# actionml/universal-recommender

Hardware: NVIDIA H100
Metric: CCO train events/sec to indicator model (higher is better)
Workload: dtype int32+f64

## Files before the change

### universal_recommender_b200/csrc/cco_api.cu

```cuda
#include <cuda_runtime.h>
#include <dlfcn.h>
#include <stdarg.h>
#include <stdio.h>
#include <stdlib.h>
#include <string.h>

#include <algorithm>
#include <charconv>
#include <cmath>
#include <functional>
#include <cub/cub.cuh>
#include <nvtx3/nvToolsExt.h>
#include <condition_variable>
#include <mutex>
#include <string>
#include <thread>
#include <unordered_map>
#include <vector>

#include "../../include/cco_b200.h"
#include "cco_kernels.cuh"
#include "cco_sampler.cuh"
#include "cco_format.cuh"
#include "cco_strings.cuh"
// ... 382 lines not shown
  c->launches++;
  ar.release(tmp);
  ar.release(kb.Alternate());
  ar.release(vb.Alternate());
  *k = kb.Current();
  *v = vb.Current();
  return CCO_OK;
}
static int bits_for(long long n) {
  int b = 1;
  while ((1LL << b) < n) ++b;
  return b;
}

static int keys_to_csr(cco_ctx *c, Arena &ar, unsigned long long *k0, unsigned long long *k1, long long n, int bits, long long n_valid,
                       long long n_rows, int32_t *col, long long *rp, long long *n_unique) {
  cudaStream_t s = c->stream;
  cub::DoubleBuffer<unsigned long long> db(k0, k1);
  size_t tb = 0;
  CK(cub::DeviceRadixSort::SortKeys(nullptr, tb, db, n, 0, bits, s));
  void *tmp;
  CKR(ar.alloc((char **)&tmp, tb));
  CK(cub::DeviceRadixSort::SortKeys(tmp, tb, db, n, 0, bits, s));
  ar.release(tmp);
  unsigned long long *sorted = db.Current(), *other = db.Alternate();
  uint32_t *flag, *pos;
  CKR(ar.alloc(&flag, n_valid + 1));
  CKR(ar.alloc(&pos, n_valid + 1));
  CK(cudaMemsetAsync(flag + n_valid, 0, 4, s));
  k_unique_flags<<<grid_for(n_valid, 256, c->sm_count), 256, 0, s>>>(n_valid, sorted, flag);
  CKR(exclusive_sum(c, ar, flag, pos, n_valid + 1));
  uint32_t nuq = 0;
  CKR(mail_fetch(c, &nuq, pos + n_valid, 4));
  k_unique_scatter<<<grid_for(n_valid, 256, c->sm_count), 256, 0, s>>>(n_valid, sorted, flag, pos, other, col);
  CKR(mail_wait(c));
  k_rowptr_from_keys<<<grid_for(n_rows + 1, 256, c->sm_count), 256, 0, s>>>(n_rows, nuq, other, rp);
  c->launches += 3;
  ar.release(flag);
  ar.release(pos);
  *n_unique = nuq;
  return CCO_OK;
}

static int canonicalize_device(cco_ctx *c, Arena &ar, DevRaw &m) {
  if (m.nnz == 0) return CCO_OK;
  unsigned long long *k0, *k1;
  CKR(ar.alloc(&k0, m.nnz));
  CKR(ar.alloc(&k1, m.nnz));
  k_expand_keys<<<grid_for(m.n_rows * kSG, 256, c->sm_count), 256, 0, c->stream>>>(m.n_rows, m.rp, m.col, k0);
  c->launches++;
  long long n_unique = 0;
  CKR(keys_to_csr(c, ar, k0, k1, m.nnz, 32 + bits_for(m.n_rows), m.nnz, m.n_rows, m.col + m.q_base, m.rp, &n_unique));
  m.col += m.q_base;
  m.q_base = 0;
  m.nnz = n_unique;
  CK(cudaGetLastError());
  ar.release(k0);
  ar.release(k1);
  return CCO_OK;
}

struct HeavyRows {
  int32_t *list = nullptr;
  int *n = nullptr;
};
static int list_heavy_rows(cco_ctx *c, Arena &ar, const DevRaw &raw, HeavyRows *h) {
  CKR(ar.alloc(&h->list, std::max<long long>(raw.n_rows, 1)));
  CKR(ar.alloc(&h->n, 1));
  CK(cudaMemsetAsync(h->n, 0, 4, c->stream));
  if (raw.n_rows > 0) {
    k_list_heavy_rows<<<grid_for(raw.n_rows, 256, c->sm_count), 256, 0, c->stream>>>(raw.n_rows, raw.rp, h->list, h->n);
    c->launches++;
  }
  return CCO_OK;
}
static void launch_check(cco_ctx *c, const DevRaw &raw, const HeavyRows &h, int *flags) {
  if (raw.n_rows <= 0) return;
  const long long q_lo = raw.q_base, q_hi = raw.q_base + raw.nnz;
  k_check_rows<kSG><<<grid_for(raw.n_rows * kSG, 256, c->sm_count), 256, 0, c->stream>>>(raw.n_rows, raw.n_cols, raw.rp, raw.col, q_lo, q_hi,
                                                                                       nullptr, nullptr, flags);
  k_check_rows<32><<<c->sm_count * 4, 256, 0, c->stream>>>(raw.n_rows, raw.n_cols, raw.rp, raw.col, q_lo, q_hi, h.list, h.n, flags);
  c->launches += 2;
}
struct SampleScratch {
  unsigned long long *col_thr = nullptr;
  uint8_t *keep = nullptr;
};
static int sample_scratch(cco_ctx *c, Arena &ar, const DevRaw &raw, const int32_t *raw_counts, int32_t m, SampleScratch *sc) {
  CKR(ar.alloc(&sc->col_thr, std::max<int32_t>(raw.n_cols, 1)));
  CKR(ar.alloc(&sc->keep, std::max<long long>(raw.nnz, 1)));
  if (raw.n_cols > 0) {
    k_col_thresholds<<<grid_for(raw.n_cols, 256, c->sm_count, 4), 256, 0, c->stream>>>(raw.n_cols, raw_counts, m, sc->col_thr);
    c->launches++;
  }
  return CCO_OK;
}
static void launch_count(cco_ctx *c, const DevRaw &raw, const SampleScratch &sc, int32_t m, int32_t seed, uint32_t flags, const int *bad,
                         uint32_t *kept, int32_t *new_counts) {
  if (raw.n_rows <= 0 || raw.nnz <= 0) return;
  const long long q_lo = raw.q_base, q_hi = raw.q_base + raw.nnz;
  const long long n_chunks = (raw.nnz + kSampleChunk - 1) / kSampleChunk;
  k_sample_count<<<grid_for(n_chunks * 32, 256, c->sm_count), 256, 0, c->stream>>>(raw.n_rows, raw.row_base, raw.rp, raw.col, raw.n_cols, q_lo, q_hi,
                                                                                  sc.col_thr, m, seed, flags, bad, kept, new_counts, sc.keep);
  c->launches++;
}
static int launch_write(cco_ctx *c, Arena &ar, const DevRaw &raw, const SampleScratch &sc, int32_t *dst) {
  if (raw.n_rows <= 0 || raw.nnz <= 0) return CCO_OK;
  long long *n_sel;
  CKR(ar.alloc(&n_sel, 1));
  size_t tb = 0;
  CK(cub::DeviceSelect::Flagged(nullptr, tb, raw.col + raw.q_base, sc.keep, dst, n_sel, (long long)raw.nnz, c->stream));
  void *tmp;
  CKR(ar.alloc((char **)&tmp, tb));
  CK(cub::DeviceSelect::Flagged(tmp, tb, raw.col + raw.q_base, sc.keep, dst, n_sel, (long long)raw.nnz, c->stream));
  ar.release(tmp);
  c->launches += 2;
  return CCO_OK;
}

constexpr int kHistCopies = 16;
static bool hist_fits_smem(const cco_ctx *c, int32_t n_cols) { return ((size_t)n_cols + 1) / 2 * 4 <= c->smem_optin; }
static int count_raw_columns(cco_ctx *c, Arena &ar, const std::vector<DevRaw> &raw, const std::vector<long long> &col_off, const cudaEvent_t *ready,
                             int *verdict, int32_t **counts_out) {
  cudaStream_t s = c->stream;
  const int n_mats = (int)raw.size();
  const long long total_cols = col_off[n_mats];
  const long long copy_stride = std::max<long long>(total_cols, 1);
  bool copies = false;
  for (int i = 0; i < n_mats; ++i) copies = copies || (raw[i].n_rows > 0 && !hist_fits_smem(c, raw[i].n_cols));
  const int n_copies = copies ? kHistCopies : 1;
  int32_t *counts;
  CKR(ar.alloc(&counts, (size_t)copy_stride * n_copies));
  CK(cudaMemsetAsync(counts, 0, sizeof(int32_t) * (size_t)copy_stride * n_copies, s));
  *counts_out = counts;
  std::vector<int> fit;
  for (int i = 0; i < n_mats; ++i)
    if (raw[i].n_rows > 0 && hist_fits_smem(c, raw[i].n_cols)) fit.push_back(i);
  for (size_t b0 = 0; b0 < fit.size(); b0 += kHistSegs) {
    const size_t b1 = std::min(fit.size(), b0 + kHistSegs);
    HistBatch hb{};
    long long nnz_sum = 0;
    int32_t max_cols = 0;
    for (size_t t = b0; t < b1; ++t) {
      nnz_sum += raw[fit[t]].nnz;
      max_cols = std::max(max_cols, raw[fit[t]].n_cols);
    }
    const size_t smem = ((size_t)max_cols + 1) / 2 * 4;
    const int per_sm = std::max(1, std::min<int>(2048 / kHistThreads, (int)(c->smem_optin / std::max<size_t>(smem + 1024, 1))));
    const long long target = (long long)c->sm_count * per_sm;
    for (size_t t = b0; t < b1; ++t) {
      const int i = fit[t];
      if (ready) CK(cudaStreamWaitEvent(s, ready[i], 0));
      const long long share = nnz_sum > 0 ? (target * raw[i].nnz + nnz_sum - 1) / nnz_sum : 1;
      const long long need = (raw[i].nnz + kHistMinEntries - 1) / kHistMinEntries;
      HistSeg &g = hb.seg[hb.n++];
      g.col = raw[i].col + raw[i].q_base;
      g.rp = raw[i].rp;
      g.nnz = raw[i].nnz;
      g.n_rows = raw[i].n_rows;
      g.q_lo = raw[i].q_base;
      g.q_hi = raw[i].q_base + raw[i].nnz;
      g.counts = counts + col_off[i];
      g.verdict = verdict ? verdict + 2 * i : nullptr;
      g.n_cols = raw[i].n_cols;
      g.cta0 = hb.cta_end;
      hb.cta_end += (int32_t)std::max(1LL, std::min(share, need));
    }
    CK(cudaFuncSetAttribute(k_col_counts_smem, cudaFuncAttributeMaxDynamicSharedMemorySize, (int)smem));
    k_col_counts_smem<<<hb.cta_end, kHistThreads, smem, s>>>(hb);
    c->launches++;
  }
  for (int i = 0; i < n_mats && copies; ++i) {
    if (raw[i].n_rows == 0 || hist_fits_smem(c, raw[i].n_cols)) continue;
    if (ready) CK(cudaStreamWaitEvent(s, ready[i], 0));
    int *v = verdict ? verdict + 2 * i : nullptr;
    if (v) {
      k_check_row_ptr<<<grid_for(raw[i].n_rows, 256, c->sm_count), 256, 0, s>>>(raw[i].n_rows, raw[i].rp, raw[i].q_base, raw[i].q_base + raw[i].nnz, v);
      c->launches++;
    }
    if (raw[i].nnz > 0) {
      k_col_histogram_flat<true><<<grid_for(raw[i].nnz, 256, c->sm_count), 256, 0, s>>>(raw[i].nnz, raw[i].col + raw[i].q_base, raw[i].n_cols,
                                                                                       counts + col_off[i], kHistCopies, copy_stride, v);
      c->launches++;
    }
  }
  if (copies) {
    k_sum_copies<<<grid_for(total_cols, 256, c->sm_count), 256, 0, s>>>(total_cols, kHistCopies, copy_stride, counts);
    c->launches++;
  }
  if (ready)
    for (int i = 0; i < n_mats; ++i) CK(cudaStreamWaitEvent(s, ready[i], 0));
  return CCO_OK;
}

static int nccl_check(int rc, const char *what) {
  if (rc != 0) return set_error(CCO_E_NCCL, "%s: %s", what, g_nccl.GetErrorString(rc));
  return CCO_OK;
}

static int downsample_all(cco_ctx *c, Arena &ar, const std::vector<DevRaw> &raw, const int *d_check , long long U,
                          const int32_t *raw_counts, int32_t *marg_all, const std::vector<long long> &col_off,
                          const cco_indicator_params_t *params, int32_t seed, uint32_t flags, std::vector<DevMat> &dm,
                          const cudaEvent_t *stage_ev ) {
  cudaStream_t s = c->stream;
  const int W = c->world, r = c->rank, n_mats = (int)raw.size();
  const long long S = (U + W - 1) / W;
  std::vector<uint32_t *> kept(n_mats, nullptr);
  std::vector<SampleScratch> sc(n_mats);
  for (int i = 0; i < n_mats; ++i) {
    DevMat *out = &dm[i];
    out->n_rows = U;
    out->n_cols = raw[i].n_cols;
    out->marg = marg_all + col_off[i];
    CKR(ar.alloc(&kept[i], (size_t)(W * S + 1)));
    CKR(ar.alloc(&out->rp, U + 1));
    CK(cudaMemsetAsync(kept[i], 0, sizeof(uint32_t) * (size_t)(W * S + 1), s));
    CKR(sample_scratch(c, ar, raw[i], raw_counts + col_off[i], params[i].max_interactions, &sc[i]));
    launch_count(c, raw[i], sc[i], params[i].max_interactions, seed, flags, d_check + 2 * i, kept[i], out->marg);
  }
  CK(cudaEventRecord(stage_ev[0], s));
  if (W > 1) {
    if (S > 0) {
      g_nccl.GroupStart();
      for (int i = 0; i < n_mats; ++i) {
        int rc = g_nccl.AllGather(kept[i] + (size_t)r * S, kept[i], (size_t)S, kNcclUint32, c->comm, s);
        if (rc != 0) { g_nccl.GroupEnd(); return nccl_check(rc, "ncclAllGather(kept counts)"); }
      }
      CKR(nccl_check(g_nccl.GroupEnd(), "ncclGroupEnd(kept counts)"));
    }
    if (col_off[n_mats] > 0)
      CKR(nccl_check(g_nccl.AllReduce(marg_all, marg_all, (size_t)col_off[n_mats], kNcclInt32, kNcclSum, c->comm, s), "ncclAllReduce(marginals)"));
  }
  std::vector<uint32_t> edge((size_t)n_mats * (W + 1), 0);
  for (int i = 0; i < n_mats; ++i) {
    CKR(exclusive_sum(c, ar, kept[i], dm[i].rp, U + 1));
    ar.release(kept[i]);
    if (W > 1)
      for (int q = 0; q <= W; ++q) CKR(mail_fetch(c, &edge[(size_t)i * (W + 1) + q], dm[i].rp + std::min<long long>((long long)q * S, U), 4));
  }
  CK(cudaEventRecord(stage_ev[1], s));
  if (W > 1) CKR(mail_wait(c));
  std::vector<long long> cap(n_mats, 0);
  std::vector<int32_t *> gathered(n_mats, nullptr);
  for (int i = 0; i < n_mats; ++i) {
    if (W == 1) {
      CKR(ar.alloc(&dm[i].col, std::max<long long>(raw[i].nnz, 1)));
      CKR(launch_write(c, ar, raw[i], sc[i], dm[i].col));
    } else {
      for (int q = 0; q < W; ++q) cap[i] = std::max<long long>(cap[i], (long long)edge[(size_t)i * (W + 1) + q + 1] - edge[(size_t)i * (W + 1) + q]);
      CKR(ar.alloc(&dm[i].col, std::max<long long>(edge[(size_t)i * (W + 1) + W], 1)));
      if (cap[i] > 0) {
        CKR(ar.alloc(&gathered[i], (size_t)(cap[i] * W)));
        CKR(launch_write(c, ar, raw[i], sc[i], gathered[i] + (size_t)r * cap[i]));
      }
    }
    ar.release(sc[i].col_thr);
    ar.release(sc[i].keep);
  }
  CK(cudaEventRecord(stage_ev[2], s));
  if (W > 1) {
    g_nccl.GroupStart();
    for (int i = 0; i < n_mats; ++i) {
      if (!gathered[i]) continue;
      int rc = g_nccl.AllGather(gathered[i] + (size_t)r * cap[i], gathered[i], (size_t)cap[i], kNcclInt32, c->comm, s);
      if (rc != 0) { g_nccl.GroupEnd(); return nccl_check(rc, "ncclAllGather(column blocks)"); }
    }
    CKR(nccl_check(g_nccl.GroupEnd(), "ncclGroupEnd(column blocks)"));
    for (int i = 0; i < n_mats; ++i) {
      if (!gathered[i]) continue;
      dim3 grid((unsigned)std::max(1, std::min(c->sm_count * 8 / W, 1024)), (unsigned)W);
      k_pack_blocks<<<grid, 256, 0, s>>>(W, S, U, cap[i], dm[i].rp, gathered[i], dm[i].col);
      c->launches++;
      ar.release(gathered[i]);
    }
  }
  CK(cudaEventRecord(stage_ev[3], s));
  CK(cudaGetLastError());
  return CCO_OK;
}


struct BinCfg {
  int group;
  int slots;
  int cap;
  int cbuf;
  int caux, keep_max, final_max;
  bool dense;
  bool bitmap;
  bool sorted;
  int bm_words;
  size_t region;
  size_t smem;
  int ctas_per_sm;
};

static int next_pow2(int x) {
  int p = 1;
  while (p < x) p <<= 1;
  return p;
}

template <int GROUP>
static int launch_rows_t(cco_ctx *c, const RowArgs &a, BinCfg &cfg, cudaStream_t st) {
  constexpr int CTA = GROUP == 32 ? 64 : GROUP;
  int occ = 1;
  void (*kern)(const RowArgs) = cfg.dense ? k_rows<GROUP, true> : k_rows<GROUP, false>;
  if constexpr (GROUP == 512 || GROUP == 256)
    if (cfg.bitmap) kern = k_rows<GROUP, false, true>;
  if constexpr (GROUP == 32)
    if (cfg.sorted) kern = k_rows<32, false, false, true>;
  CK(cudaFuncSetAttribute(kern, cudaFuncAttributeMaxDynamicSharedMemorySize, (int)cfg.smem));
  CK(cudaOccupancyMaxActiveBlocksPerMultiprocessor(&occ, kern, CTA, cfg.smem));
  kern<<<c->sm_count * std::max(occ, 1) * 4, CTA, cfg.smem, st>>>(a);
  cfg.ctas_per_sm = occ;
  c->launches++;
  CK(cudaGetLastError());
  return CCO_OK;
}
static int launch_rows(cco_ctx *c, const RowArgs &a, BinCfg &cfg, cudaStream_t st) {
  switch (cfg.group) {
    case 1024: return launch_rows_t<1024>(c, a, cfg, st);
    case 512: return launch_rows_t<512>(c, a, cfg, st);
    case 256: return launch_rows_t<256>(c, a, cfg, st);
    case 128: return launch_rows_t<128>(c, a, cfg, st);
    case 32: return launch_rows_t<32>(c, a, cfg, st);
  }
  return set_error(CCO_E_INVALID_ARG, "internal: bad bin config");
}

static BinCfg make_cfg(cco_ctx *c, int group, int want_slots, int top_k, int n_cols_b) {
  BinCfg f;
  const int groups = group == 32 ? 2 : 1;
  f.group = group;
  f.final_max = next_pow2(top_k);
  f.cbuf = next_pow2(top_k + std::max(group, 128) + (group == 32 ? 64 : 0));
  if (group == 32 && top_k + 32 <= 96) f.cbuf = 128;
  f.keep_max = std::max(f.final_max, (f.cbuf - group) / 2);
  f.caux = group == 32 ? 0 : f.keep_max;
  size_t fixed = (size_t)(f.cbuf + f.caux) * 16 + 2 * 256 + 512 + 1024 + (size_t)(group / 32) * 256;
  size_t avail = (c->smem_optin - 1024) / groups;
// ... 5101 lines not shown
    if (len[i] < 1 || len[i] > 32) return set_error(CCO_E_CUDA, "text %lld has length %d", (long long)i, len[i]);
    memcpy(bytes + offsets[i], slot.data() + 32 * (size_t)i, (size_t)len[i]);
    offsets[i + 1] = offsets[i] + len[i];
  }
  return CCO_OK;
}

int cco_debug_downsample(cco_ctx_t *c, const cco_csr_t *m, int32_t max_interactions, int32_t seed, uint32_t flags,
                         int64_t **row_ptr, int32_t **col_idx, int32_t *raw_col_counts, int32_t *new_col_counts) {
  if (!c || !m || !row_ptr || !col_idx) return set_error(CCO_E_INVALID_ARG, "null argument");
  if (c->world != 1 || !c->members.empty()) return set_error(CCO_E_UNSUPPORTED, "debug entries need a single-GPU context");
  cco_indicator_params_t prm = {max_interactions, 1, 0, 0.0};
  CKR(validate_host(1, m, &prm));
  CK(cudaSetDevice(c->device));
  mail_reset(c);
  c->ev_timing_used = c->ev_plain_used = 0;
  cco_dataset *ds = nullptr;
  CKR(dataset_upload(c, 1, m, flags, &ds));
  struct DG { cco_dataset *d; ~DG() { dataset_release(d); } } dg{ds};
  Arena ar(c->stream);
  Prepared p;
  CKR(prepare(c, ar, ds, &prm, seed, flags, &p));
  const DevMat &dm = p.dm[0];
  std::vector<uint32_t> rp32((size_t)m->n_rows + 1);
  CK(cudaMemcpyAsync(rp32.data(), dm.rp, sizeof(uint32_t) * rp32.size(), cudaMemcpyDeviceToHost, c->stream));
  if (raw_col_counts && m->n_cols > 0)
    CK(cudaMemcpyAsync(raw_col_counts, p.raw_counts, sizeof(int32_t) * (size_t)m->n_cols, cudaMemcpyDeviceToHost, c->stream));
  if (new_col_counts && m->n_cols > 0)
    CK(cudaMemcpyAsync(new_col_counts, dm.marg, sizeof(int32_t) * (size_t)m->n_cols, cudaMemcpyDeviceToHost, c->stream));
  CK(cudaStreamSynchronize(c->stream));
  CK(cudaGetLastError());
  size_t nnz = rp32[m->n_rows];
  int64_t *rp = (int64_t *)malloc(sizeof(int64_t) * rp32.size());
  int32_t *ci = (int32_t *)calloc(std::max<size_t>(nnz, 1), sizeof(int32_t));
  if (!rp || !ci) return set_error(CCO_E_OOM, "malloc failed");
  for (size_t i = 0; i < rp32.size(); ++i) rp[i] = rp32[i];
  const size_t n_copy = std::min<size_t>(nnz, (size_t)ds->nnz[0]);
  if (n_copy) CK(cudaMemcpy(ci, dm.col, sizeof(int32_t) * n_copy, cudaMemcpyDeviceToHost));
  *row_ptr = rp;
  *col_idx = ci;
  return CCO_OK;
}

int cco_debug_downsample_block(cco_ctx_t *c, const cco_csr_t *m, int64_t row_lo, int64_t row_hi, const int32_t *raw_col_counts,
                               int32_t max_interactions, int32_t seed, uint32_t flags, int64_t *kept_per_row, int32_t **col_idx,
                               int32_t *new_col_counts) {
  if (!c || !m || !col_idx || (m->n_rows > 0 && !kept_per_row) || (m->n_cols > 0 && (!raw_col_counts || !new_col_counts)))
    return set_error(CCO_E_INVALID_ARG, "null argument");
  if (c->world != 1 || !c->members.empty()) return set_error(CCO_E_UNSUPPORTED, "debug entries need a single-GPU context");
  cco_indicator_params_t prm = {max_interactions, 1, 0, 0.0};
  CKR(validate_host(1, m, &prm));
  if (row_lo < 0 || row_hi < row_lo || row_hi > m->n_rows)
    return set_error(CCO_E_INVALID_ARG, "rows [%lld, %lld) outside [0, %lld)", (long long)row_lo, (long long)row_hi, (long long)m->n_rows);
  CK(cudaSetDevice(c->device));
  mail_reset(c);
  cudaStream_t s = c->stream;
  cco_dataset *ds = nullptr;
  CKR(dataset_upload(c, 1, m, flags, &ds));
  struct DG { cco_dataset *d; ~DG() { dataset_release(d); } } dg{ds};
  Arena ar(s);
  const long long U = ds->n_users;
  const int32_t width = std::max<int32_t>(m->n_cols, 1);
  long long q[2] = {0, 0};
  CK(cudaMemcpyAsync(&q[0], ds->rp[0] + row_lo, sizeof(long long), cudaMemcpyDeviceToHost, s));
  CK(cudaMemcpyAsync(&q[1], ds->rp[0] + row_hi, sizeof(long long), cudaMemcpyDeviceToHost, s));
  CK(cudaStreamSynchronize(s));
  DevRaw blk;
  blk.n_rows = row_hi - row_lo;
  blk.row_base = row_lo;
  blk.n_cols = m->n_cols;
  blk.q_base = q[0];
  blk.nnz = q[1] - q[0];
  blk.rp = ds->rp[0] + row_lo;
  blk.col = ds->col[0];
  int32_t *counts, *marg, *dst;
  uint32_t *kept;
  CKR(ar.alloc(&counts, width));
  CKR(ar.alloc(&marg, width));
  CKR(ar.alloc(&kept, U + 1));
  CKR(ar.alloc(&dst, std::max<long long>(blk.nnz, 1)));
  if (m->n_cols > 0) CK(cudaMemcpyAsync(counts, raw_col_counts, sizeof(int32_t) * (size_t)m->n_cols, cudaMemcpyHostToDevice, s));
  CK(cudaMemsetAsync(marg, 0, sizeof(int32_t) * (size_t)width, s));
  CK(cudaMemsetAsync(kept, 0, sizeof(uint32_t) * ((size_t)U + 1), s));
  SampleScratch sc;
  CKR(sample_scratch(c, ar, blk, counts, max_interactions, &sc));
  launch_count(c, blk, sc, max_interactions, seed, flags, nullptr, kept, marg);
  CKR(launch_write(c, ar, blk, sc, dst));
  std::vector<uint32_t> hk((size_t)U + 1);
  CK(cudaMemcpyAsync(hk.data(), kept, sizeof(uint32_t) * hk.size(), cudaMemcpyDeviceToHost, s));
  if (m->n_cols > 0) CK(cudaMemcpyAsync(new_col_counts, marg, sizeof(int32_t) * (size_t)m->n_cols, cudaMemcpyDeviceToHost, s));
  CK(cudaStreamSynchronize(s));
  CK(cudaGetLastError());
  size_t n_kept = 0;
  for (long long r = 0; r < U; ++r) {
    kept_per_row[r] = hk[r];
    if (r >= row_lo && r < row_hi) n_kept += hk[r];
  }
  int32_t *ci = (int32_t *)calloc(std::max<size_t>(n_kept, 1), sizeof(int32_t));
  if (!ci) return set_error(CCO_E_OOM, "malloc failed");
  const size_t n_copy = std::min<size_t>(n_kept, (size_t)blk.nnz);
  if (n_copy) {
    cudaError_t e = cudaMemcpy(ci, dst, sizeof(int32_t) * n_copy, cudaMemcpyDeviceToHost);
    if (e != cudaSuccess) {
      free(ci);
      return set_error(CCO_E_CUDA, "cudaMemcpy: %s", cudaGetErrorString(e));
    }
  }
  *col_idx = ci;
  return CCO_OK;
}

int cco_debug_cooccurrence(cco_ctx_t *c, const cco_csr_t *a, const cco_csr_t *b, int64_t **row_ptr, int32_t **col_idx,
                           int32_t **count) {
  if (!c || !a || !b || !row_ptr || !col_idx || !count) return set_error(CCO_E_INVALID_ARG, "null argument");
  if (c->world != 1 || !c->members.empty()) return set_error(CCO_E_UNSUPPORTED, "debug entries need a single-GPU context");
  cco_csr_t two[2] = {*a, *b};
  cco_indicator_params_t prm[2] = {{0x7fffffff, 1, 0, 0.0}, {0x7fffffff, 1, 0, 0.0}};
  CKR(validate_host(2, two, prm));
  CK(cudaSetDevice(c->device));
  mail_reset(c);
  c->ev_timing_used = c->ev_plain_used = 0;
  cco_dataset *ds = nullptr;
  CKR(dataset_upload(c, 2, two, 0, &ds));
  struct DG { cco_dataset *d; ~DG() { dataset_release(d); } } dg{ds};
  Arena ar(c->stream);
  struct CopyJoin {
    cco_ctx *c;
    ~CopyJoin() { cudaStreamSynchronize(c->copy_stream); }
  } copy_join{c};
  Prepared prep;
  CKR(prepare(c, ar, ds, prm, 0, 0, &prep));
  const int32_t n_items_a = prep.dm[0].n_cols;
  ResultMat rm;
  IndicatorOut io;
  IndicatorState ist;
  struct EG { IndicatorState &x; ~EG() { if (x.packed) cudaEventDestroy(x.packed); } } eg{ist};
  cco_indicator_params_t p1 = {0x7fffffff, 1, 0, 0.0};
  auto put = [&]() {
    for (void *p : {(void *)rm.row_ptr, (void *)rm.col, (void *)rm.llr, (void *)rm.cnt})
      if (p) c->pinned_put(p);
  };
  int rc = enqueue_indicator(c, ar, prep.at_ptr, prep.at_users, n_items_a, prep.dm[0].marg, prep.max_marg[0], prep.max_marg[1], prep.dm[1],
                             a->n_rows, false, p1, 0, true, nullptr, nullptr, nullptr, &ist);
  if (rc == CCO_OK) rc = finish_indicator(c, &ist, 0, 0, &rm, &io);
  cudaStreamSynchronize(c->copy_stream);
  if (rc != CCO_OK) {
    put();
    return rc;
  }
  size_t nnz = (size_t)rm.row_ptr[n_items_a];
  int64_t *rp = (int64_t *)malloc(sizeof(int64_t) * ((size_t)n_items_a + 1));
  int32_t *ci = (int32_t *)malloc(sizeof(int32_t) * std::max<size_t>(nnz, 1));
  int32_t *cn = (int32_t *)malloc(sizeof(int32_t) * std::max<size_t>(nnz, 1));
  if (!rp || !ci || !cn) {
    put();
    return set_error(CCO_E_OOM, "malloc failed");
  }
  memcpy(rp, rm.row_ptr, sizeof(int64_t) * ((size_t)n_items_a + 1));
  std::vector<std::pair<int32_t, int32_t>> tmp;
  for (int32_t r = 0; r < n_items_a; ++r) {
    size_t lo = (size_t)rp[r], hi = (size_t)rp[r + 1];
    tmp.resize(hi - lo);
    for (size_t q = lo; q < hi; ++q) tmp[q - lo] = {rm.col[q], rm.cnt[q]};
    std::sort(tmp.begin(), tmp.end());
    for (size_t q = lo; q < hi; ++q) {
      ci[q] = tmp[q - lo].first;
      cn[q] = tmp[q - lo].second;
    }
  }
  put();
// ... 983 lines not shown
```

### universal_recommender_b200/csrc/cco_sampler.cuh

```cuda
#pragma once

#include <cuda_runtime.h>
#include <stdint.h>

#include "cco_kernels.cuh"

namespace cco {

constexpr int kSampleChunk = 256;

template <typename P>
__device__ __forceinline__ long long warp_find_row(const P *__restrict__ rp, long long n_rows, long long q, int lane) {
  long long lo = 0, hi = n_rows;
  while (hi - lo > 1) {
    const long long step = (hi - lo + 31) / 32;
    const long long p = lo + lane * step;
    const bool ok = p < hi && (long long)rp[p] <= q;
    const unsigned b = __ballot_sync(0xffffffffu, ok) | 1u;
    const int top = 31 - __clz(b);
    lo += top * step;
    hi = hi < lo + step ? hi : lo + step;
  }
  return lo;
}

__global__ void __launch_bounds__(256) k_sample_count(long long n_rows, long long row_base, const long long *__restrict__ rp,
                                                      const int32_t *__restrict__ col, int32_t n_cols, long long q_lo, long long q_hi,
                                                      const unsigned long long *__restrict__ col_thr, int32_t m, int32_t seed, uint32_t flags,
                                                      const int *__restrict__ bad ,
                                                      uint32_t *__restrict__ kept_per_row , int32_t *__restrict__ new_counts,
                                                      uint8_t *__restrict__ keep_flag) {
  const int lane = threadIdx.x & 31;
  const long long warp = (blockIdx.x * (long long)blockDim.x + threadIdx.x) >> 5;
  const long long n_warps = ((long long)gridDim.x * blockDim.x) >> 5;
  const long long n_chunks = (q_hi - q_lo + kSampleChunk - 1) / kSampleChunk;
  const bool intdiv = (flags & CCO_FLAG_ROWRATE_INTDIV) != 0;
  const long long kNoRow = 0x7fffffffffffffffLL;
  if (n_rows <= 0) return;
  if (bad && *bad) {
    for (long long q = blockIdx.x * (long long)blockDim.x + threadIdx.x; q < q_hi - q_lo; q += (long long)gridDim.x * blockDim.x) keep_flag[q] = 0;
    return;
  }
  for (long long chunk = warp; chunk < n_chunks; chunk += n_warps) {
    const long long Q0 = q_lo + chunk * kSampleChunk;
    const long long Q1 = Q0 + kSampleChunk < q_hi ? Q0 + kSampleChunk : q_hi;
    long long base = warp_find_row(rp, n_rows, Q0, lane);
    long long start_i, end_i;
    unsigned long long t_i, x_i;
    uint32_t kept_i;
#define CCO_LOAD_WINDOW()                                                                                   \
  {                                                                                                         \
    const long long r = base + lane;                                                                        \
    start_i = end_i = kNoRow;                                                                               \
    t_i = kKeepAlways;                                                                                      \
    x_i = 0;                                                                                                \
    if (r < n_rows) {                                                                                       \
      start_i = rp[r];                                                                                      \
      end_i = rp[r + 1];                                                                                    \
      const long long d = end_i - start_i;                                                                  \
      if (d > (long long)m) t_i = rate_threshold(row_sample_rate(d, m, intdiv));  \
      x_i = mix64(((uint64_t)(uint32_t)seed << 32) | (uint64_t)(uint32_t)(row_base + r));                   \
    }                                                                                                       \
    kept_i = 0;                                                                                             \
  }
#define CCO_FLUSH_WINDOW()                                                                                  \
  if (kept_i) atomicAdd(&kept_per_row[row_base + base + lane], kept_i);
    CCO_LOAD_WINDOW()
    for (long long qb = Q0; qb < Q1; qb += 32) {
      const long long q = qb + lane;
      bool pending = q < Q1;
      const int32_t j = pending ? col[q] : 0;
      unsigned long long t_col = kKeepAlways;
      if (pending && (uint32_t)j < (uint32_t)n_cols) t_col = col_thr[j];
      while (true) {
        int idx = 0;
#pragma unroll
        for (int step = 16; step > 0; step >>= 1) {
          const long long v = __shfl_sync(0xffffffffu, end_i, idx + step - 1);
          if (v <= q) idx += step;
        }
        {
          const long long v = __shfl_sync(0xffffffffu, end_i, idx);
          if (v <= q) idx += 1;
        }
        const int src = idx & 31;
        const unsigned long long t_row = __shfl_sync(0xffffffffu, t_i, src);
        const unsigned long long x_row = __shfl_sync(0xffffffffu, x_i, src);
        const bool here = pending && idx < 32;
        const bool real_row = base + idx < n_rows;
        bool keep = false;
        if (here) {
          keep = real_row && (uint32_t)j < (uint32_t)n_cols && keep_entry_thr(t_row, t_col, x_row, (uint32_t)j);
          keep_flag[q - q_lo] = keep ? 1 : 0;
          if (keep && new_counts) atomicAdd(&new_counts[j], 1);
        }
        const unsigned kb = __ballot_sync(0xffffffffu, keep);
        const int a = start_i <= qb ? 0 : (start_i >= qb + 32 ? 32 : (int)(start_i - qb));
        const int b = end_i <= qb ? 0 : (end_i >= qb + 32 ? 32 : (int)(end_i - qb));
        if (b > a) {
          const unsigned below_b = b >= 32 ? 0xffffffffu : ((1u << b) - 1u);
          const unsigned below_a = (1u << a) - 1u;
          kept_i += __popc(kb & below_b & ~below_a);
        }
        pending = pending && !here;
        if (!__any_sync(0xffffffffu, pending)) break;
        CCO_FLUSH_WINDOW()
        base += 32;
        if (base >= n_rows) {
          if (pending) keep_flag[q - q_lo] = 0;
          kept_i = 0;
          start_i = end_i = kNoRow;
          break;
        }
        CCO_LOAD_WINDOW()
      }
      if (base >= n_rows) {
        for (long long q2 = qb + 32 + lane; q2 < Q1; q2 += 32) keep_flag[q2 - q_lo] = 0;
        break;
      }
    }
    if (base < n_rows && base + lane < n_rows) { CCO_FLUSH_WINDOW() }
#undef CCO_LOAD_WINDOW
#undef CCO_FLUSH_WINDOW
  }
}

__global__ void k_check_row_ptr(long long n_rows, const long long *__restrict__ rp, long long q_lo, long long q_hi, int *flags) {
  int bad = 0;
  for (long long r = blockIdx.x * (long long)blockDim.x + threadIdx.x; r < n_rows; r += (long long)gridDim.x * blockDim.x) {
    const long long s = rp[r], e = rp[r + 1];
    if (e < s || s < q_lo || e > q_hi) bad = 1;
  }
  if (bad) atomicOr(&flags[0], 1);
}
template <bool AGG>
__global__ void k_col_histogram_flat(long long n, const int32_t *__restrict__ col, int32_t n_cols, int32_t *__restrict__ counts, int n_copies,
                                     long long copy_stride, int *flags ) {
  int32_t *mine = counts + (long long)(blockIdx.x % n_copies) * copy_stride;
  const int lane = threadIdx.x & 31;
  int bad = 0;
  for (long long q0 = blockIdx.x * (long long)blockDim.x + (threadIdx.x & ~31); q0 < n; q0 += (long long)gridDim.x * blockDim.x) {
    const long long q = q0 + lane;
    const bool act = q < n;
    const int32_t j = act ? col[q] : -1;
    const bool ok = act && (uint32_t)j < (uint32_t)n_cols;
    if (act && !ok) bad = 1;
    if (AGG) {
      const unsigned om = __ballot_sync(0xffffffffu, ok);
      if (ok) {
        const unsigned peers = __match_any_sync(om, j);
        if ((__ffs(peers) - 1) == lane) atomicAdd(&mine[j], __popc(peers));
      }
    } else if (ok) {
      atomicAdd(&mine[j], 1);
    }
  }
  if (flags && bad) atomicOr(&flags[0], 1);
}

__global__ void __launch_bounds__(256) k_transpose_entries(long long n_rows, const uint32_t *__restrict__ rp, const int32_t *__restrict__ col,
                                                           uint32_t *__restrict__ cursor, int32_t *__restrict__ users) {
  if (n_rows <= 0) return;
  const int lane = threadIdx.x & 31;
  const long long warp = (blockIdx.x * (long long)blockDim.x + threadIdx.x) >> 5;
  const long long n_warps = ((long long)gridDim.x * blockDim.x) >> 5;
  const long long nnz = rp[n_rows];
  const long long n_chunks = (nnz + kSampleChunk - 1) / kSampleChunk;
  for (long long chunk = warp; chunk < n_chunks; chunk += n_warps) {
    const long long Q0 = chunk * kSampleChunk;
    const long long Q1 = Q0 + kSampleChunk < nnz ? Q0 + kSampleChunk : nnz;
    long long base = warp_find_row(rp, n_rows, Q0, lane);
    long long end_i = base + lane < n_rows ? (long long)rp[base + lane + 1] : 0x7fffffffffffffffLL;
    for (long long qb = Q0; qb < Q1; qb += 32) {
      const long long q = qb + lane;
      bool pending = q < Q1;
      const int32_t j = pending ? col[q] : 0;
      while (true) {
        int idx = 0;
#pragma unroll
        for (int step = 16; step > 0; step >>= 1) {
          const long long v = __shfl_sync(0xffffffffu, end_i, idx + step - 1);
          if (v <= q) idx += step;
        }
        if (__shfl_sync(0xffffffffu, end_i, idx & 31) <= q) idx += 1;
        const bool here = pending && idx < 32;
        if (here) users[atomicAdd(&cursor[j], 1u)] = (int32_t)(base + idx);
        pending = pending && !here;
        if (!__any_sync(0xffffffffu, pending)) break;
        base += 32;
        end_i = base + lane < n_rows ? (long long)rp[base + lane + 1] : 0x7fffffffffffffffLL;
      }
    }
  }
}

constexpr int kHistSegs = 8;
constexpr int kHistThreads = 1024;
constexpr long long kHistMinEntries = 1 << 16;
struct HistSeg {
  const int32_t *col;
  const long long *rp;
  long long nnz, n_rows, q_lo, q_hi;
  int32_t *counts;
  int *verdict;
  int32_t n_cols;
  int32_t cta0;
// ... 52 lines not shown
```

Baseline: 4.655 billion.

## Replace byte keep-flags and CUB select with chunk bitmasks and batched sample kernels

The sampler now writes a packed keep bitmask and a per-chunk kept count instead of a byte flag per entry. A second custom kernel compacts the kept columns using a prefix sum over chunk counts, replacing the two-call cub::DeviceSelect::Flagged. Up to eight matrices are batched into one threshold launch and one count launch through a struct of segments. The count kernel also preloads the chunk's column ids into registers and prefetches column thresholds. This cuts flag traffic and launches, at the cost of more register use and a linear segment lookup per chunk.

New measurement: 4.690 billion (median of 6 runs). No clear change (+0.8%).

```diff
diff --git a/universal_recommender_b200/csrc/cco_api.cu b/universal_recommender_b200/csrc/cco_api.cu
--- a/universal_recommender_b200/csrc/cco_api.cu
+++ b/universal_recommender_b200/csrc/cco_api.cu
@@ -488,40 +488,69 @@
   k_check_rows<32><<<c->sm_count * 4, 256, 0, c->stream>>>(raw.n_rows, raw.n_cols, raw.rp, raw.col, q_lo, q_hi, h.list, h.n, flags);
   c->launches += 2;
 }
-struct SampleScratch {
+struct SamplePlan {
+  std::vector<SampleBatch> batch;
   unsigned long long *col_thr = nullptr;
-  uint8_t *keep = nullptr;
+  uint32_t *bits = nullptr, *chunk_kept = nullptr, *chunk_base = nullptr;
+  long long n_chunks = 0;
 };
-static int sample_scratch(cco_ctx *c, Arena &ar, const DevRaw &raw, const int32_t *raw_counts, int32_t m, SampleScratch *sc) {
-  CKR(ar.alloc(&sc->col_thr, std::max<int32_t>(raw.n_cols, 1)));
-  CKR(ar.alloc(&sc->keep, std::max<long long>(raw.nnz, 1)));
-  if (raw.n_cols > 0) {
-    k_col_thresholds<<<grid_for(raw.n_cols, 256, c->sm_count, 4), 256, 0, c->stream>>>(raw.n_cols, raw_counts, m, sc->col_thr);
-    c->launches++;
-  }
-  return CCO_OK;
-}
-static void launch_count(cco_ctx *c, const DevRaw &raw, const SampleScratch &sc, int32_t m, int32_t seed, uint32_t flags, const int *bad,
-                         uint32_t *kept, int32_t *new_counts) {
-  if (raw.n_rows <= 0 || raw.nnz <= 0) return;
-  const long long q_lo = raw.q_base, q_hi = raw.q_base + raw.nnz;
-  const long long n_chunks = (raw.nnz + kSampleChunk - 1) / kSampleChunk;
-  k_sample_count<<<grid_for(n_chunks * 32, 256, c->sm_count), 256, 0, c->stream>>>(raw.n_rows, raw.row_base, raw.rp, raw.col, raw.n_cols, q_lo, q_hi,
-                                                                                  sc.col_thr, m, seed, flags, bad, kept, new_counts, sc.keep);
-  c->launches++;
-}
-static int launch_write(cco_ctx *c, Arena &ar, const DevRaw &raw, const SampleScratch &sc, int32_t *dst) {
-  if (raw.n_rows <= 0 || raw.nnz <= 0) return CCO_OK;
-  long long *n_sel;
-  CKR(ar.alloc(&n_sel, 1));
-  size_t tb = 0;
-  CK(cub::DeviceSelect::Flagged(nullptr, tb, raw.col + raw.q_base, sc.keep, dst, n_sel, (long long)raw.nnz, c->stream));
-  void *tmp;
-  CKR(ar.alloc((char **)&tmp, tb));
-  CK(cub::DeviceSelect::Flagged(tmp, tb, raw.col + raw.q_base, sc.keep, dst, n_sel, (long long)raw.nnz, c->stream));
-  ar.release(tmp);
-  c->launches += 2;
-  return CCO_OK;
+static int sample_pass1(cco_ctx *c, Arena &ar, const std::vector<DevRaw> &raw, const int32_t *raw_counts, const std::vector<long long> &col_off,
+                        const int32_t *m, int32_t seed, uint32_t flags, const int *bad, const std::vector<uint32_t *> &kept, int32_t *new_counts,
+                        SamplePlan *p) {
+  cudaStream_t s = c->stream;
+  const int n_mats = (int)raw.size();
+  CKR(ar.alloc(&p->col_thr, (size_t)std::max<long long>(col_off[n_mats], 1)));
+  for (int i = 0; i < n_mats; ++i) {
+    if (i % kSampleSegs == 0) p->batch.emplace_back();
+    SampleBatch &b = p->batch.back();
+    SampleSeg &g = b.seg[b.n++];
+    const DevRaw &r = raw[i];
+    g.rp = r.rp;
+    g.col = r.col;
+    g.raw_counts = raw_counts + col_off[i];
+    g.col_thr = p->col_thr + col_off[i];
+    g.kept = kept[i];
+    g.new_counts = new_counts ? new_counts + col_off[i] : nullptr;
+    g.bad = bad ? bad + 2 * i : nullptr;
+    g.n_rows = r.n_rows;
+    g.row_base = r.row_base;
+    g.q_lo = r.q_base;
+    g.q_hi = r.q_base + r.nnz;
+    g.chunk0 = p->n_chunks;
+    g.col0 = b.col_end;
+    g.n_cols = r.n_cols;
+    g.m = m[i];
+    if (r.n_rows > 0 && r.nnz > 0) p->n_chunks += (r.nnz + kSampleChunk - 1) / kSampleChunk;
+    b.chunk_end = p->n_chunks;
+    b.col_end += r.n_cols;
+  }
+  CKR(ar.alloc(&p->bits, (size_t)std::max<long long>(p->n_chunks * kChunkWords, 1)));
+  CKR(ar.alloc(&p->chunk_kept, (size_t)p->n_chunks + 1));
+  CKR(ar.alloc(&p->chunk_base, (size_t)p->n_chunks + 1));
+  CK(cudaMemsetAsync(p->chunk_kept + p->n_chunks, 0, 4, s));
+  for (const SampleBatch &b : p->batch) {
+    if (b.col_end > 0) {
+      k_col_thresholds_batch<<<grid_for(b.col_end, 256, c->sm_count, 4), 256, 0, s>>>(b);
+      c->launches++;
+    }
+    const long long n = b.chunk_end - b.seg[0].chunk0;
+    if (n > 0) {
+      k_sample_count<<<grid_for(n * 32, 256, c->sm_count), 256, 0, s>>>(b, seed, flags, p->bits, p->chunk_kept);
+      c->launches++;
+    }
+  }
+  return exclusive_sum(c, ar, p->chunk_kept, p->chunk_base, p->n_chunks + 1);
+}
+static void sample_pass2(cco_ctx *c, SamplePlan &p, const std::vector<int32_t *> &dst) {
+  int i = 0;
+  for (SampleBatch &b : p.batch) {
+    for (int k = 0; k < b.n; ++k) b.seg[k].dst = dst[i++];
+    const long long n = b.chunk_end - b.seg[0].chunk0;
+    if (n > 0) {
+      k_sample_write<<<grid_for(n * 32, 256, c->sm_count), 256, 0, c->stream>>>(b, p.bits, p.chunk_base);
+      c->launches++;
+    }
+  }
 }
 
 constexpr int kHistCopies = 16;
@@ -612,18 +641,19 @@
   const int W = c->world, r = c->rank, n_mats = (int)raw.size();
   const long long S = (U + W - 1) / W;
   std::vector<uint32_t *> kept(n_mats, nullptr);
-  std::vector<SampleScratch> sc(n_mats);
+  std::vector<int32_t> m(n_mats);
   for (int i = 0; i < n_mats; ++i) {
     DevMat *out = &dm[i];
     out->n_rows = U;
     out->n_cols = raw[i].n_cols;
     out->marg = marg_all + col_off[i];
+    m[i] = params[i].max_interactions;
     CKR(ar.alloc(&kept[i], (size_t)(W * S + 1)));
     CKR(ar.alloc(&out->rp, U + 1));
     CK(cudaMemsetAsync(kept[i], 0, sizeof(uint32_t) * (size_t)(W * S + 1), s));
-    CKR(sample_scratch(c, ar, raw[i], raw_counts + col_off[i], params[i].max_interactions, &sc[i]));
-    launch_count(c, raw[i], sc[i], params[i].max_interactions, seed, flags, d_check + 2 * i, kept[i], out->marg);
-  }
+  }
+  SamplePlan plan;
+  CKR(sample_pass1(c, ar, raw, raw_counts, col_off, m.data(), seed, flags, d_check, kept, marg_all, &plan));
   CK(cudaEventRecord(stage_ev[0], s));
   if (W > 1) {
     if (S > 0) {
@@ -647,22 +677,22 @@
   CK(cudaEventRecord(stage_ev[1], s));
   if (W > 1) CKR(mail_wait(c));
   std::vector<long long> cap(n_mats, 0);
-  std::vector<int32_t *> gathered(n_mats, nullptr);
+  std::vector<int32_t *> gathered(n_mats, nullptr), dst(n_mats, nullptr);
   for (int i = 0; i < n_mats; ++i) {
     if (W == 1) {
       CKR(ar.alloc(&dm[i].col, std::max<long long>(raw[i].nnz, 1)));
-      CKR(launch_write(c, ar, raw[i], sc[i], dm[i].col));
+      dst[i] = dm[i].col;
     } else {
       for (int q = 0; q < W; ++q) cap[i] = std::max<long long>(cap[i], (long long)edge[(size_t)i * (W + 1) + q + 1] - edge[(size_t)i * (W + 1) + q]);
       CKR(ar.alloc(&dm[i].col, std::max<long long>(edge[(size_t)i * (W + 1) + W], 1)));
       if (cap[i] > 0) {
         CKR(ar.alloc(&gathered[i], (size_t)(cap[i] * W)));
-        CKR(launch_write(c, ar, raw[i], sc[i], gathered[i] + (size_t)r * cap[i]));
+        dst[i] = gathered[i] + (size_t)r * cap[i];
       }
     }
-    ar.release(sc[i].col_thr);
-    ar.release(sc[i].keep);
-  }
+  }
+  sample_pass2(c, plan, dst);
+  for (void *b : {(void *)plan.col_thr, (void *)plan.bits, (void *)plan.chunk_kept, (void *)plan.chunk_base}) ar.release(b);
   CK(cudaEventRecord(stage_ev[2], s));
   if (W > 1) {
     g_nccl.GroupStart();
@@ -5930,10 +5960,9 @@
   if (m->n_cols > 0) CK(cudaMemcpyAsync(counts, raw_col_counts, sizeof(int32_t) * (size_t)m->n_cols, cudaMemcpyHostToDevice, s));
   CK(cudaMemsetAsync(marg, 0, sizeof(int32_t) * (size_t)width, s));
   CK(cudaMemsetAsync(kept, 0, sizeof(uint32_t) * ((size_t)U + 1), s));
-  SampleScratch sc;
-  CKR(sample_scratch(c, ar, blk, counts, max_interactions, &sc));
-  launch_count(c, blk, sc, max_interactions, seed, flags, nullptr, kept, marg);
-  CKR(launch_write(c, ar, blk, sc, dst));
+  SamplePlan plan;
+  CKR(sample_pass1(c, ar, {blk}, counts, {0, (long long)m->n_cols}, &max_interactions, seed, flags, nullptr, {kept}, marg, &plan));
+  sample_pass2(c, plan, {dst});
   std::vector<uint32_t> hk((size_t)U + 1);
   CK(cudaMemcpyAsync(hk.data(), kept, sizeof(uint32_t) * hk.size(), cudaMemcpyDeviceToHost, s));
   if (m->n_cols > 0) CK(cudaMemcpyAsync(new_col_counts, marg, sizeof(int32_t) * (size_t)m->n_cols, cudaMemcpyDeviceToHost, s));
diff --git a/universal_recommender_b200/csrc/cco_sampler.cuh b/universal_recommender_b200/csrc/cco_sampler.cuh
--- a/universal_recommender_b200/csrc/cco_sampler.cuh
+++ b/universal_recommender_b200/csrc/cco_sampler.cuh
@@ -24,104 +24,167 @@
   return lo;
 }
 
-__global__ void __launch_bounds__(256) k_sample_count(long long n_rows, long long row_base, const long long *__restrict__ rp,
-                                                      const int32_t *__restrict__ col, int32_t n_cols, long long q_lo, long long q_hi,
-                                                      const unsigned long long *__restrict__ col_thr, int32_t m, int32_t seed, uint32_t flags,
-                                                      const int *__restrict__ bad ,
-                                                      uint32_t *__restrict__ kept_per_row , int32_t *__restrict__ new_counts,
-                                                      uint8_t *__restrict__ keep_flag) {
+constexpr int kSampleSegs = 8;
+constexpr int kChunkWords = kSampleChunk / 32;
+struct SampleSeg {
+  const long long *rp;
+  const int32_t *col;
+  const int32_t *raw_counts;
+  unsigned long long *col_thr;
+  uint32_t *kept;
+  int32_t *new_counts;
+  const int *bad;
+  int32_t *dst;
+  long long n_rows, row_base, q_lo, q_hi;
+  long long chunk0;
+  long long col0;
+  int32_t n_cols, m;
+};
+struct SampleBatch {
+  SampleSeg seg[kSampleSegs];
+  int32_t n;
+  long long chunk_end;
+  long long col_end;
+};
+
+__global__ void k_col_thresholds_batch(const SampleBatch b) {
+  for (long long g = blockIdx.x * (long long)blockDim.x + threadIdx.x; g < b.col_end; g += (long long)gridDim.x * blockDim.x) {
+    int i = 0;
+    while (i + 1 < b.n && g >= b.seg[i + 1].col0) ++i;
+    const SampleSeg &s = b.seg[i];
+    const long long j = g - s.col0;
+    const int32_t c = s.raw_counts[j];
+    s.col_thr[j] = c <= s.m ? kKeepAlways : rate_threshold(__ddiv_rn((double)s.m, (double)c));
+  }
+}
+
+__device__ __forceinline__ int sample_seg_of(const SampleBatch &b, long long chunk) {
+  int i = 0;
+  while (i + 1 < b.n && chunk >= b.seg[i + 1].chunk0) ++i;
+  return i;
+}
+__device__ __forceinline__ int chunk_rel(long long v, long long Q0) {
+  const long long d = v - Q0;
+  return d <= 0 ? 0 : (d >= kSampleChunk ? kSampleChunk : (int)d);
+}
+
+__global__ void __launch_bounds__(256) k_sample_count(const SampleBatch b, int32_t seed, uint32_t flags, uint32_t *__restrict__ bits,
+                                                      uint32_t *__restrict__ chunk_kept) {
   const int lane = threadIdx.x & 31;
   const long long warp = (blockIdx.x * (long long)blockDim.x + threadIdx.x) >> 5;
   const long long n_warps = ((long long)gridDim.x * blockDim.x) >> 5;
-  const long long n_chunks = (q_hi - q_lo + kSampleChunk - 1) / kSampleChunk;
   const bool intdiv = (flags & CCO_FLAG_ROWRATE_INTDIV) != 0;
-  const long long kNoRow = 0x7fffffffffffffffLL;
-  if (n_rows <= 0) return;
-  if (bad && *bad) {
-    for (long long q = blockIdx.x * (long long)blockDim.x + threadIdx.x; q < q_hi - q_lo; q += (long long)gridDim.x * blockDim.x) keep_flag[q] = 0;
-    return;
-  }
-  for (long long chunk = warp; chunk < n_chunks; chunk += n_warps) {
-    const long long Q0 = q_lo + chunk * kSampleChunk;
-    const long long Q1 = Q0 + kSampleChunk < q_hi ? Q0 + kSampleChunk : q_hi;
-    long long base = warp_find_row(rp, n_rows, Q0, lane);
-    long long start_i, end_i;
+  for (long long chunk = b.seg[0].chunk0 + warp; chunk < b.chunk_end; chunk += n_warps) {
+    const SampleSeg &s = b.seg[sample_seg_of(b, chunk)];
+    const long long n_rows = s.n_rows, row_base = s.row_base;
+    const int32_t n_cols = s.n_cols, m = s.m;
+    const long long Q0 = s.q_lo + (chunk - s.chunk0) * kSampleChunk;
+    const int n_q = (int)(s.q_hi - Q0 < kSampleChunk ? s.q_hi - Q0 : kSampleChunk);
+    uint32_t my_word = 0, n_kept = 0;
+    if (s.bad && *s.bad) {
+      if (lane < kChunkWords) bits[chunk * kChunkWords + lane] = 0;
+      if (lane == 0) chunk_kept[chunk] = 0;
+      continue;
+    }
+    int32_t jq[kChunkWords];
+#pragma unroll
+    for (int k = 0; k < kChunkWords; ++k) jq[k] = 32 * k + lane < n_q ? s.col[Q0 + 32 * k + lane] : 0;
+    unsigned long long t_next = lane < n_q && (uint32_t)jq[0] < (uint32_t)n_cols ? s.col_thr[jq[0]] : kKeepAlways;
+    long long base = warp_find_row(s.rp, n_rows, Q0, lane);
+    int start_i, end_i;
     unsigned long long t_i, x_i;
     uint32_t kept_i;
 #define CCO_LOAD_WINDOW()                                                                                   \
   {                                                                                                         \
     const long long r = base + lane;                                                                        \
-    start_i = end_i = kNoRow;                                                                               \
+    start_i = end_i = kSampleChunk;                                                                         \
     t_i = kKeepAlways;                                                                                      \
     x_i = 0;                                                                                                \
     if (r < n_rows) {                                                                                       \
-      start_i = rp[r];                                                                                      \
-      end_i = rp[r + 1];                                                                                    \
-      const long long d = end_i - start_i;                                                                  \
+      const long long a = s.rp[r], e = s.rp[r + 1];                                                         \
+      start_i = chunk_rel(a, Q0);                                                                           \
+      end_i = chunk_rel(e, Q0);                                                                             \
+      const long long d = e - a;                                                                            \
       if (d > (long long)m) t_i = rate_threshold(row_sample_rate(d, m, intdiv));  \
       x_i = mix64(((uint64_t)(uint32_t)seed << 32) | (uint64_t)(uint32_t)(row_base + r));                   \
     }                                                                                                       \
     kept_i = 0;                                                                                             \
   }
 #define CCO_FLUSH_WINDOW()                                                                                  \
-  if (kept_i) atomicAdd(&kept_per_row[row_base + base + lane], kept_i);
+  if (kept_i) atomicAdd(&s.kept[row_base + base + lane], kept_i);
     CCO_LOAD_WINDOW()
-    for (long long qb = Q0; qb < Q1; qb += 32) {
-      const long long q = qb + lane;
-      bool pending = q < Q1;
-      const int32_t j = pending ? col[q] : 0;
-      unsigned long long t_col = kKeepAlways;
-      if (pending && (uint32_t)j < (uint32_t)n_cols) t_col = col_thr[j];
+    for (int qb = 0; qb < n_q; qb += 32) {
+      const int q = qb + lane;
+      bool pending = q < n_q;
+      const int32_t j = jq[0];
+      const unsigned long long t_col = t_next;
+#pragma unroll
+      for (int k = 0; k + 1 < kChunkWords; ++k) jq[k] = jq[k + 1];
+      jq[kChunkWords - 1] = 0;
+      t_next = q + 32 < n_q && (uint32_t)jq[0] < (uint32_t)n_cols ? s.col_thr[jq[0]] : kKeepAlways;
+      unsigned word = 0;
       while (true) {
         int idx = 0;
 #pragma unroll
-        for (int step = 16; step > 0; step >>= 1) {
-          const long long v = __shfl_sync(0xffffffffu, end_i, idx + step - 1);
-          if (v <= q) idx += step;
-        }
-        {
-          const long long v = __shfl_sync(0xffffffffu, end_i, idx);
-          if (v <= q) idx += 1;
-        }
+        for (int step = 16; step > 0; step >>= 1)
+          if (__shfl_sync(0xffffffffu, end_i, idx + step - 1) <= q) idx += step;
+        if (__shfl_sync(0xffffffffu, end_i, idx) <= q) idx += 1;
         const int src = idx & 31;
         const unsigned long long t_row = __shfl_sync(0xffffffffu, t_i, src);
         const unsigned long long x_row = __shfl_sync(0xffffffffu, x_i, src);
         const bool here = pending && idx < 32;
         const bool real_row = base + idx < n_rows;
-        bool keep = false;
-        if (here) {
-          keep = real_row && (uint32_t)j < (uint32_t)n_cols && keep_entry_thr(t_row, t_col, x_row, (uint32_t)j);
-          keep_flag[q - q_lo] = keep ? 1 : 0;
-          if (keep && new_counts) atomicAdd(&new_counts[j], 1);
-        }
+        const bool keep = here && real_row && (uint32_t)j < (uint32_t)n_cols && keep_entry_thr(t_row, t_col, x_row, (uint32_t)j);
+        if (keep && s.new_counts) atomicAdd(&s.new_counts[j], 1);
         const unsigned kb = __ballot_sync(0xffffffffu, keep);
-        const int a = start_i <= qb ? 0 : (start_i >= qb + 32 ? 32 : (int)(start_i - qb));
-        const int b = end_i <= qb ? 0 : (end_i >= qb + 32 ? 32 : (int)(end_i - qb));
-        if (b > a) {
-          const unsigned below_b = b >= 32 ? 0xffffffffu : ((1u << b) - 1u);
+        word |= kb;
+        const int a = min(max(start_i - qb, 0), 32), e = min(max(end_i - qb, 0), 32);
+        if (e > a) {
+          const unsigned below_e = e >= 32 ? 0xffffffffu : ((1u << e) - 1u);
           const unsigned below_a = (1u << a) - 1u;
-          kept_i += __popc(kb & below_b & ~below_a);
+          kept_i += __popc(kb & below_e & ~below_a);
         }
         pending = pending && !here;
         if (!__any_sync(0xffffffffu, pending)) break;
         CCO_FLUSH_WINDOW()
         base += 32;
         if (base >= n_rows) {
-          if (pending) keep_flag[q - q_lo] = 0;
           kept_i = 0;
-          start_i = end_i = kNoRow;
+          start_i = end_i = kSampleChunk;
           break;
         }
         CCO_LOAD_WINDOW()
       }
-      if (base >= n_rows) {
-        for (long long q2 = qb + 32 + lane; q2 < Q1; q2 += 32) keep_flag[q2 - q_lo] = 0;
-        break;
-      }
+      if (lane == (qb >> 5)) my_word = word;
+      n_kept += __popc(word);
+      if (base >= n_rows) break;
     }
     if (base < n_rows && base + lane < n_rows) { CCO_FLUSH_WINDOW() }
 #undef CCO_LOAD_WINDOW
 #undef CCO_FLUSH_WINDOW
+    if (lane < kChunkWords) bits[chunk * kChunkWords + lane] = my_word;
+    if (lane == 0) chunk_kept[chunk] = n_kept;
+  }
+}
+
+__global__ void __launch_bounds__(256) k_sample_write(const SampleBatch b, const uint32_t *__restrict__ bits,
+                                                      const uint32_t *__restrict__ chunk_base) {
+  const int lane = threadIdx.x & 31;
+  const long long warp = (blockIdx.x * (long long)blockDim.x + threadIdx.x) >> 5;
+  const long long n_warps = ((long long)gridDim.x * blockDim.x) >> 5;
+  const unsigned below = (1u << lane) - 1u;
+  for (long long chunk = b.seg[0].chunk0 + warp; chunk < b.chunk_end; chunk += n_warps) {
+    const SampleSeg &s = b.seg[sample_seg_of(b, chunk)];
+    const long long Q0 = s.q_lo + (chunk - s.chunk0) * kSampleChunk;
+    const uint32_t w = lane < kChunkWords ? bits[chunk * kChunkWords + lane] : 0u;
+    uint32_t at = chunk_base[chunk] - chunk_base[s.chunk0];
+    int32_t *dst = s.dst;
+#pragma unroll
+    for (int k = 0; k < kChunkWords; ++k) {
+      const unsigned word = __shfl_sync(0xffffffffu, w, k);
+      if ((word >> lane) & 1u) dst[at + __popc(word & below)] = s.col[Q0 + k * 32 + lane];
+      at += __popc(word);
+    }
   }
 }
 
```
